# p-mc-grath/DMMFODS

Measured on AMD Instinct MI355X. Metric: training images/sec at 1280x1920 RGB+LiDAR, higher is better.
Workload: dtype f16; 1 GPU; C2 d121 early-fusion 6ch b4 1280x1920; key=c2, per_gpu_batch=4, global_batch=4, height=1280, width=1920, storage_dtype=fp16, accumulate=fp32, parallelism=dp1, weights=random-init (reference init, seed 123)

## Files before the change

dmmfods_amd/_lib.py:

```python
import ctypes as C
import os

_HERE = os.path.dirname(os.path.abspath(__file__))
LIB_PATH = os.environ.get("DMM_LIB_PATH") or os.path.join(_HERE, "libdmmfods_hip.so")

DMM_F32, DMM_F16, DMM_BF16 = 0, 1, 2
LOSS_BCE, LOSS_FOCAL = 0, 1
T_CONV, T_CONVT, T_BN_WEIGHT, T_BN_BIAS, T_BN_MEAN, T_BN_VAR, T_BN_TRACKED = range(7)
ERR_INVALID, ERR_SHAPE, ERR_HIP, ERR_STATE, ERR_NO_DEVICE = -1, -2, -3, -4, -5


class ModelDesc(C.Structure):
    _fields_ = [
        ("growth_rate", C.c_int32), ("num_blocks", C.c_int32), ("block_config", C.c_int32 * 8),
        ("num_init_features", C.c_int32), ("bn_size", C.c_int32), ("num_classes", C.c_int32),
        ("concat_before_block_num", C.c_int32), ("stream_1_in_channels", C.c_int32),
        ("stream_2_in_channels", C.c_int32), ("batch", C.c_int32), ("height", C.c_int32), ("width", C.c_int32),
        ("dtype", C.c_int32), ("loss_scale", C.c_float), ("bn_momentum", C.c_float), ("bn_eps", C.c_float),
        ("iou_threshold", C.c_float), ("use_mfma", C.c_int32),
    ]


class ConvDesc(C.Structure):
    _fields_ = [(n, C.c_int32) for n in (
# ... 24 lines not shown
    if not os.path.exists(LIB_PATH):
        raise ImportError(
            f"{LIB_PATH} is missing: build it with `python -c 'import __graft_entry__ as g; g.build()'` "
            "(or `make -C dmmfods_amd/csrc`).  dmmfods_amd has no CPU fallback.")
    import torch
    tl = os.path.join(os.path.dirname(torch.__file__), "lib", "libamdhip64.so")
    if os.path.exists(tl):
        C.CDLL(tl, mode=C.RTLD_GLOBAL)
    L = C.CDLL(LIB_PATH)
    vp, i32, i64, f32, sz = C.c_void_p, C.c_int32, C.c_int64, C.c_float, C.c_size_t
    L.dmm_last_error.restype = C.c_char_p
    L.dmm_version.restype = C.c_int
    L.dmm_last_impl.restype = C.c_int
    L.dmm_impl_name.restype = C.c_char_p
    L.dmm_impl_name.argtypes = [C.c_int]
    L.dmm_impl_mask.restype = C.c_uint
    L.dmm_impl_mask.argtypes = [C.c_int]
    L.dmm_set_option.restype = C.c_int
    L.dmm_set_option.argtypes = [C.c_char_p, C.c_int]
    L.dmm_plan_create.argtypes = [C.POINTER(ModelDesc), C.POINTER(vp)]
    L.dmm_plan_destroy.argtypes = [vp]
    L.dmm_plan_destroy.restype = C.c_int
    L.dmm_plan_num_tensors.argtypes = [vp]
    L.dmm_plan_tensor_info.argtypes = [vp, C.c_int, C.POINTER(C.c_char_p), C.POINTER(i32), C.POINTER(i32),
                                       C.POINTER(i64 * 4), C.POINTER(i64)]
    L.dmm_plan_num_params.argtypes = [vp]
    L.dmm_plan_num_params.restype = i64
    L.dmm_plan_num_buffer_elems.argtypes = [vp]
    L.dmm_plan_num_buffer_elems.restype = i64
    L.dmm_plan_workspace_bytes.argtypes = [vp]
# ... 33 lines not shown
    L.dmm_conv_wgrad_ex.argtypes = [C.POINTER(ConvDesc), vp, vp, vp, vp, vp, vp, vp, C.c_int, vp, vp, vp]
    L.dmm_conv_dgrad_ex.argtypes = [C.POINTER(ConvDesc), vp, vp, vp, vp, vp, vp, vp, vp, vp, C.c_int, vp, vp, vp]
    L.dmm_conv1x1_backward_fused.argtypes = [C.POINTER(ConvDesc), vp, vp, vp, vp, vp, vp, vp, vp, vp, C.c_int, vp, vp, vp, vp]
    L.dmm_conv5_wgrad_stats.argtypes = [C.POINTER(ConvDesc), vp, vp, vp, vp, vp, vp, vp, vp, vp]
    _lib = L
    return L


EXPORTS = [
    "dmm_last_error", "dmm_version", "dmm_set_option", "dmm_plan_create", "dmm_plan_destroy", "dmm_plan_num_tensors",
    "dmm_plan_tensor_info", "dmm_plan_num_params", "dmm_plan_num_buffer_elems", "dmm_plan_workspace_bytes",
    "dmm_plan_forward_flops", "dmm_plan_bind", "dmm_plan_forward", "dmm_plan_loss_backward", "dmm_plan_backward",
    "dmm_plan_loss_metrics", "dmm_plan_num_graph_replays", "dmm_plan_set_loss", "dmm_loss_forward", "dmm_plan_num_grad_buckets", "dmm_plan_grad_bucket",
    "dmm_plan_grad_bucket_wait", "dmm_plan_profile_begin", "dmm_plan_profile_filter", "dmm_plan_profile_num_ops", "dmm_plan_profile_op",
    "dmm_plan_profile_collect", "dmm_adam_step", "dmm_conv_scratch_bytes", "dmm_conv_forward", "dmm_conv_wgrad",
    "dmm_conv_dgrad", "dmm_conv_wgrad_ex", "dmm_conv_dgrad_ex", "dmm_conv1x1_backward_fused", "dmm_conv5_wgrad_stats", "dmm_last_impl", "dmm_impl_name", "dmm_impl_mask",
    "dmm_grad_guard_scratch_bytes", "dmm_guard_state_init", "dmm_adam_step_guarded", "dmm_grad_sumsq", "dmm_plan_set_dynamic_loss_scale",
]


def check(rc):
    if rc == 0:
        return
    msg = lib().dmm_last_error().decode(errors="replace")
    if rc == ERR_SHAPE:
        raise ValueError(msg)
    if rc == ERR_INVALID and "fusion" in msg:
        raise AttributeError(msg)
    if rc == ERR_INVALID:
        raise ValueError(msg)
    raise DmmError(f"dmm status {rc}: {msg}")
# ... 17 lines not shown
```

dmmfods_amd/csrc/capi.cpp:

```cpp
#include <algorithm>
#include <atomic>
#include <cmath>
#include <cstdio>
#include <cstdlib>
#include <cstring>
#include <stdexcept>
#include <chrono>
#include <mutex>
#include <string>
#include <unistd.h>

#include "dispatch.h"
#include "plan.h"

using namespace dmm;

void plan_build_tables(dmm_plan* p);
void plan_bind(dmm_plan* p, void* ws);

static thread_local std::string g_err;
static int fail(int code, const std::string& msg) {
  g_err = msg;
  return code;
}
#define HIPCHK(expr)                                                                                   \
  do {                                                                                                 \
    hipError_t e__ = (expr);                                                                           \
    if (e__ != hipSuccess) return fail(DMM_ERR_HIP, std::string(#expr) + ": " + hipGetErrorString(e__)); \
  } while (0)

static bool g_overlap_wgrad = getenv("DMM_NO_OVERLAP") == nullptr;
static int g_graph = getenv("DMM_GRAPH") ? std::max(1, atoi(getenv("DMM_GRAPH"))) : 0;
static unsigned long long g_option_epoch = 1;
static int g_bucket_mb = getenv("DMM_GRAD_BUCKET_MB") ? atoi(getenv("DMM_GRAD_BUCKET_MB")) : 25;
static std::atomic<unsigned> g_family_off{lab_family_off()};
static unsigned plan_deny(const dmm_plan* p) { return (p->sw.no_hf ? 1u << IMPL_HF : 0u) | g_family_off; }

namespace {
struct DevicePool {
  std::mutex mu;
  hipStream_t side = nullptr, pack = nullptr, capture = nullptr;
  std::vector<hipEvent_t> free_plain, free_timing;
  long events_made = 0;
};
constexpr int MAX_DEVICES = 64;
DevicePool* g_pools[MAX_DEVICES] = {};
std::mutex g_pools_mu;

DevicePool* pool_of(int device) {
  if (device < 0 || device >= MAX_DEVICES) return nullptr;
// ... 49 lines not shown

const char* dmm_last_error(void) { return g_err.c_str(); }
int dmm_version(void) { return 101; }

static const char* const kImplNames[IMPL_COUNT] = {"auto", "generic", "thin", "conv3", "cvp", "halo", "wg3", "wg5", "wgp", "pig", "bw1", "hf", "cf", "wgpw", "cvw"};
static const struct { const char* option; int family; } kFamilyOptions[] = {
    {"thin_logits", IMPL_THIN}, {"conv3", IMPL_CONV3}, {"wg3", IMPL_WG3}, {"wgp", IMPL_WGP},
    {"wg5", IMPL_WG5},          {"cvp", IMPL_CVP},     {"bw1", IMPL_BW1}, {"pig", IMPL_PIG},
};

int dmm_set_option(const char* name, int value) {
  if (!name) return fail(DMM_ERR_INVALID, "null argument");
  ++g_option_epoch;
  if (std::string(name) == "overlap_wgrad") { g_overlap_wgrad = value != 0; return DMM_OK; }
  if (std::string(name) == "graph") { g_graph = value; return DMM_OK; }
  for (const auto& o : kFamilyOptions)
    if (std::string(name) == o.option) {
      if (value != 0) g_family_off &= ~(1u << o.family);
      else g_family_off |= 1u << o.family;
      return DMM_OK;
    }
  if (std::string(name) == "grad_bucket_mb") {
    if (value < 0) return fail(DMM_ERR_INVALID, "grad_bucket_mb must be >= 0");
    g_bucket_mb = value;
    return DMM_OK;
  }
  return fail(DMM_ERR_INVALID, std::string("unknown option ") + name);
}

int dmm_plan_create(const dmm_model_desc* desc, dmm_plan** out) {
// ... 655 lines not shown
  const size_t dg = (size_t)((d->R * d->S * rup(d->Cout, 8) + g.BK - 1) / g.BK + 16) * rup(d->Cin, 128) * g.BK * g.esz;
  return fwd + dg + 2 * dg + (size_t)rup(d->Cout, 8) * 8 + 8192 + (size_t)W5_SBUF64_FLOATS * sizeof(float);
}

static void fill_one_seg(Seg& s, const dmm_conv_desc* d, const OneConv& g, const void* x, const float* scale, const float* shift,
                         const std::vector<Tap>& taps) {
  memset(&s, 0, sizeof(s));
  s.src = x; s.ld = g.Cst; s.Hs = d->H; s.Ws = d->W; s.C = g.Cst; s.Cpad = g.Cst;
  s.mode = d->transposed ? 0 : d->mode;
  s.istride = g.istride;
  if (d->bn_relu) { s.scale = scale; s.shift = shift; }
  fill_seg_taps(s, taps, g.BK);
}

int dmm_last_impl(void) { return g_last_impl; }
unsigned dmm_impl_mask(int reset) { const unsigned m = g_impl_mask; if (reset) g_impl_mask = 0; return m; }
const char* dmm_impl_name(int impl) { return impl >= 0 && impl < IMPL_COUNT ? kImplNames[impl] : "?"; }

int dmm_conv_forward(const dmm_conv_desc* d, const void* x, const float* w, const float* scale, const float* shift, void* y,
                     double* stats, void* scratch, void* stream) {
  OneConv g;
  if (!d || !geometry(d, g)) return fail(DMM_ERR_INVALID, "unsupported conv descriptor");
  hipStream_t st = (hipStream_t)stream;
  std::vector<PackDesc> packs;
  std::vector<int> prefix;
  PackDesc* dd; int* dp; int total_rows;
  layout_fwd(d, g, (uint8_t*)scratch, w, nullptr, packs, &dd, &dp, prefix, total_rows);
  HIPCHK(upload(dd, packs.data(), packs.size() * sizeof(PackDesc), st));
  HIPCHK(upload(dp, prefix.data(), prefix.size() * sizeof(int), st));
  HIPCHK(hipStreamSynchronize(st));
// ... 84 lines not shown
    HIPCHK(hipMemsetAsync(dw, 0, wn * sizeof(float), st));
    HIPCHK(launch_unpack(dd, dp, 1, pd.seg[0].nchunks * pd.Npad, d->dtype, 1.0f, st));
    return DMM_OK;
  }
  std::vector<PackDesc> packs;
  std::vector<int> prefix;
  PackDesc* dd; int* dp; int total_rows;
  const size_t used = layout_fwd(d, g, (uint8_t*)scratch, dw , dw, packs, &dd, &dp, prefix, total_rows);
  Scratch S{(uint8_t*)scratch, used};
  float* zeros = (float*)S.take((size_t)rup(d->Cout, 8) * sizeof(float) + 64);
  if (S.off > dmm_conv_scratch_bytes(d)) return fail(DMM_ERR_INVALID, "scratch too small");
  HIPCHK(hipMemsetAsync(scratch, 0, S.off, st));
  HIPCHK(upload(dd, packs.data(), packs.size() * sizeof(PackDesc), st));
  HIPCHK(upload(dp, prefix.data(), prefix.size() * sizeof(int), st));
  HIPCHK(hipStreamSynchronize(st));
  for (size_t ph = 0; ph < packs.size(); ++ph) {
    WgradArgs a;
    memset(&a, 0, sizeof(a));
    a.nseg = 1;
    fill_one_seg(a.seg[0], d, g, x, scale, shift, g.phase_taps[ph]);
    a.B = d->B; a.Ho = g.Ho; a.Wo = g.Wo; a.M = d->B * g.Ho * g.Wo;
    a.dy.src = dy; a.dy.ld = d->Cout; a.dy.Hs = g.Hout; a.dy.Ws = g.Wout; a.dy.C = rup(d->Cout, 8); a.dy.Cpad = a.dy.C;
    a.dy.mode = G_PLAIN; a.dy.istride = g.ostride; a.dy.ntaps = 1; a.dy.nchunks = 1;
    a.dy.taps[0] = (short)((g.phase_xy[ph].first & 0xff) | ((g.phase_xy[ph].second & 0xff) << 8));
    set_eff_grad(a.dy, yfwd, d->Cout, q, r, zeros);
    a.N = d->Cout; a.Npad = packs[ph].Npad;
    a.dpack = (float*)packs[ph].dpack;
    HIPCHK(launch_wgrad(a, d->dtype, d->use_mfma != 0, st, IMPL_AUTO, g_family_off));
  }
  HIPCHK(hipMemsetAsync(dw, 0, wn * sizeof(float), st));
  HIPCHK(launch_unpack(dd, dp, (int)packs.size(), total_rows, d->dtype, 1.0f, st));
  return DMM_OK;
}

int dmm_conv5_wgrad_stats(const dmm_conv_desc* d, const void* x, const void* dy, const float* w, const float* scale, const float* shift,
                          float* dw, double* red, void* scratch, void* stream) {
  OneConv g;
  if (!d || !geometry(d, g)) return fail(DMM_ERR_INVALID, "unsupported conv descriptor");
  if (d->transposed || d->mode != 0 || d->stride != 1 || d->R != 5 || d->S != 5 || d->pad != 2 || !d->bn_relu || d->Cin != 64 || d->Cout > 4 ||
      d->dtype == DMM_F32 || !d->use_mfma)
    return fail(DMM_ERR_INVALID, "serves the 5x5 convolution of 64 channels onto <= 4 behind BN+ReLU in 16-bit storage");
  hipStream_t st = (hipStream_t)stream;
  const size_t wn = (size_t)d->Cin * d->Cout * 25;
  const std::vector<Tap> taps = taps_conv_dgrad(5, 5, 2);
// ... 161 lines not shown
```

dmmfods_amd/csrc/common.h:

```cpp
#pragma once
#include <hip/hip_runtime.h>
#include <stddef.h>
#include <stdint.h>
#include <stdlib.h>

namespace dmm {

typedef _Float16 f16;
typedef f16 f16x8 __attribute__((ext_vector_type(8)));
typedef f16 f16x4 __attribute__((ext_vector_type(4)));
typedef __bf16 bf16;
typedef bf16 bf16x8 __attribute__((ext_vector_type(8)));
typedef bf16 bf16x4 __attribute__((ext_vector_type(4)));
typedef bf16 bf16x2 __attribute__((ext_vector_type(2)));
typedef float f32x4 __attribute__((ext_vector_type(4)));
typedef float f32x16 __attribute__((ext_vector_type(16)));

enum DType { DT_F32 = 0, DT_F16 = 1, DT_BF16 = 2 };
static inline size_t dtype_size(int dt) { return dt == DT_F32 ? 4 : 2; }

template <typename T> struct TT;
template <> struct TT<float> {
  static constexpr int SLOT = 4;
  typedef f32x4 vec;
// ... 80 lines not shown
  Seg dy;
  int N, Npad;
  float* dpack;
  int rows_per_split;
  int kgroups;
  float* part;
  int part_slots;
  int nphase;
  short ph_xtaps[4][4];
  short ph_ytap[4];
  float* ph_dpack[4];
  const float* t_mean;
  const float* t_invstd;
  float* sbuf;
  signed char ph_ntaps[4];
};
struct RawFinArgs {
  const float* sbuf;
  float* dpack;
  int Npad;
  const float* w;
  int Kin, koff, nreal;
  int tapw[9];
  const float* gamma;
  const float* beta;
  double* red1;
  double* red2;
};
constexpr int W5_SBUF_FLOATS = 5 * 64 * 32;
struct Fin64Args {
  const float* sbuf;
// ... 63 lines not shown
```

dmmfods_amd/csrc/plan.cpp:

```cpp
#include "plan.h"

#include <algorithm>
#include <cmath>
#include <cstdio>
#include <cstdlib>
#include <cstring>
#include <map>
#include <stdexcept>

namespace dmm {

static unsigned tw1(int mt) { return 0xffffff00u | (unsigned)mt; }

std::vector<Tap> taps_conv(int R, int S, int pad) {
  std::vector<Tap> t;
  for (int ky = 0; ky < R; ++ky)
    for (int kx = 0; kx < S; ++kx) t.push_back({ky - pad, kx - pad, tw1(ky * S + kx)});
  return t;
}
std::vector<Tap> taps_conv_dgrad(int R, int S, int pad) {
  std::vector<Tap> t;
  for (int ky = 0; ky < R; ++ky)
    for (int kx = 0; kx < S; ++kx) t.push_back({pad - ky, pad - kx, tw1(ky * S + kx)});
  return t;
// ... 741 lines not shown
      const PackDesc& pd = P.packs[ph.pack];
      a.N = c.N; a.Npad = pd.Npad;
      a.dpack = (float*)pd.dpack;
      const double np = (double)c.phases.size();
      o.impl = wgrad_pick(a, dtype, d.use_mfma != 0, deny);
      tag(o, ncls(o.impl, ROLE_WGRAD, pd.Npad), short_name(c.wname), conv_flops(c, c.phases.size()) * (wseg < c.nseg ? (double)c.seg[0].Cw / c.Kin : 1.0),
          (src_bytes(c) + grad_reads(c) * out_bytes(c)) / np + w_bytes(c) * 4.0 / esz / np);
    }
    if (c.phases.size() == 4 && wseg == 1 && !P.sw.no_wgp_merge)
      merge_last_four_phases(
          [](const Op& po, const Op& f) {
            const int nt = po.w.seg[0].ntaps;
            return po.kind == OP_WGRAD && po.impl == IMPL_WGP && po.w.nseg == 1 && (nt == 1 || nt == 2 || nt == 4) && po.w.seg[0].src == f.w.seg[0].src &&
                   po.w.dy.src == f.w.dy.src;
          },
          [](Op& m, const Op& po, int ph) {
            m.w.nphase = 4;
            for (int t = 0; t < 4; ++t) m.w.ph_xtaps[ph][t] = po.w.seg[0].taps[t < po.w.seg[0].ntaps ? t : 0];
            m.w.ph_ntaps[ph] = (signed char)po.w.seg[0].ntaps;
            m.w.ph_ytap[ph] = po.w.dy.taps[0];
            m.w.ph_dpack[ph] = po.w.dpack;
          },
          [&](Op& m) {
            bool all4 = true;
            for (int ph = 0; ph < 4; ++ph) all4 = all4 && m.w.ph_ntaps[ph] == 4;
            if (all4) m.w.ph_ntaps[0] = m.w.ph_ntaps[1] = m.w.ph_ntaps[2] = m.w.ph_ntaps[3] = 0;
            return wgrad_pick(m.w, dtype, d.use_mfma != 0, deny) == IMPL_WGP;
          });
  }

  bool raw_segment_once(const ConvRec& c) const {
    return c.nseg == 2 && c.phases.size() == 4 && c.shared_master && c.seg[1].C == 8 && c.seg[1].istride == 2 && c.ostride == 2 &&
           !lab_flag("DMM_NO_RAW_ONCE");
  }
  void emit_wgrad_raw(ConvRec& c, ConvBwd& st) {
    const Buf& ob = bufs[c.obuf];
    const SegRec& sr = c.seg[1];
    float* raw_sbuf = nullptr;
    if (dtype != DT_F32 && c.N == 64 && !P.sw.no_raw_stats) raw_sbuf = zbptr<float>(W5_SBUF_FLOATS);
    Op& o = push(OP_WGRAD);
    WgradArgs& a = o.w;
// ... 711 lines not shown
};

}
}

using namespace dmm;

PlanSwitches PlanSwitches::from_environment() {
  PlanSwitches s;
  auto on = [](const char* n) { const char* v = getenv(n); return v != nullptr && !(v[0] == '0' && v[1] == 0); };
  s.no_pack_tiles = on("DMM_NO_PACK_TILES");
  s.no_hf = on("DMM_NO_HF");
  s.no_c3_merge = on("DMM_NO_C3_MERGE");
  s.no_cvp_merge = on("DMM_NO_CVP_MERGE");
  s.no_wgp_merge = on("DMM_NO_WGP_MERGE");
  s.no_two_pass = on("DMM_NO_TWO_PASS");
  s.no_eff_compact = on("DMM_NO_EFF_COMPACT");
  s.no_s2_interleave = on("DMM_NO_S2_INTERLEAVE");
  s.no_raw_stats = on("DMM_NO_RAW_STATS");
  s.no_r1_stats = on("DMM_NO_R1_STATS");
  const char* pc = getenv("DMM_PACK_CUT");
  s.pack_cut = pc ? std::max(1, atoi(pc)) : 0;
  return s;
}

void plan_build_tables(dmm_plan* p) {
  build_tensor_table(p->desc, p->tensors, p->nparams, p->nbuf);
  Builder b(*p, true, nullptr);
  b.build();
  b.emit_all();
// ... 39 lines not shown
```

dmmfods_amd/csrc/plan.h:

```cpp
#pragma once
#include <cstring>
#include <stdexcept>
#include <string>
#include <vector>

#include "../../include/dmmfods_hip.h"
#include "common.h"
#include "pointwise.h"

namespace dmm {

struct plan_sizing_error : std::runtime_error { using std::runtime_error::runtime_error; };

struct TensorInfo {
  std::string name;
  int kind, ndim;
  int64_t shape[4];
  int64_t off;
};

struct Tap {
  int dy, dx;
  unsigned tapw;
};
// ... 45 lines not shown
    RawFinArgs rf;
    Fin64Args f64;
  };
  Op() { memset(static_cast<void*>(this), 0, sizeof(*this)); signal = -1; impl = IMPL_AUTO; }
};

}

struct GradBucket {
  int64_t off = 0, n = 0;
  int ev_main = -1, ev_side = -1;
  int ready = -1;
};

struct PlanSwitches {
  bool no_pack_tiles = false, no_hf = false, no_c3_merge = false, no_cvp_merge = false, no_wgp_merge = false, no_two_pass = false,
       no_eff_compact = false, no_s2_interleave = false, no_raw_stats = false, no_r1_stats = false;
  int pack_cut = 0;
  static PlanSwitches from_environment();
};

struct dmm_plan {
  dmm_model_desc desc;
  PlanSwitches sw;
  unsigned deny = 0;
  std::vector<dmm::TensorInfo> tensors;
  int64_t nparams = 0, nbuf = 0;
  size_t zero_bytes = 0, zero_bwd_bytes = 0, main_bytes = 0;
  double fwd_flops = 0;
  bool bound = false;
  void* ws = nullptr;
// ... 42 lines not shown
```

dmmfods_amd/csrc/wgp.hip:

```cpp
#include <algorithm>
#include <cstdio>
#include <cstdlib>

#include "common.h"
#include "dispatch.h"
#include "gather.h"
#include "isa.h"

namespace dmm {

constexpr int WP_TH = 8, WP_TW = 16;
constexpr int WP_HH = 9, WP_HWR = 17;
constexpr int WP_HW = 20;
constexpr int WP_CA = 128;
constexpr int WP_X_BYTES = WP_HH * WP_HW * 256;
constexpr int WP_Y_BYTES = BM * 256;
constexpr int WP_LDS = WP_X_BYTES + WP_Y_BYTES;

struct WgpArgs {
  WgradArgs w;
  int tiles_y, tiles_x, ntiles, tiles_per_wg, nsplit;
  int nct, ncot;
  int dymin, dxmin;
  int ph_dymin[4], ph_dxmin[4];
// ... 175 lines not shown
  const int r = lane & 31, h = lane >> 5;
  const int cpt = sx.Cpad / 32;
#pragma unroll
  for (int t = 0; t < NTAP; ++t) {
    const size_t chunk = (size_t)t * cpt + ct * 4 + wave;
#pragma unroll
    for (int j = 0; j < NJ; ++j)
#pragma unroll
      for (int i = 0; i < 16; ++i) {
        const int n = cot * NCO + 32 * j + (i & 3) + 8 * (i >> 2) + 4 * h;
        atomic_add_f32(dpack_ + (chunk * a.Npad + n) * 32 + r, acc[t][j][i]);
      }
  }
}

bool wgpw_resolve(const WgradArgs& a, int dtype, int ntap, int nj, const WgpGeom& q, Resolved& r);
hipError_t wgpw_launch(const Resolved& r, hipStream_t st);

template <typename T>
static LdsLauncher<WgpArgs> wgp_instance(int ntap, int nj, int pq) {
  if (ntap == 4 && nj == 2) return pq ? launch_lds<wgp_kernel<T, 4, 2, 2>, WgpArgs> : launch_lds<wgp_kernel<T, 4, 2, 0>, WgpArgs>;
  if (ntap == 2 && nj == 4) return pq ? launch_lds<wgp_kernel<T, 2, 4, 2>, WgpArgs> : launch_lds<wgp_kernel<T, 2, 4, 0>, WgpArgs>;
  if (ntap == 2 && nj == 2) return pq ? launch_lds<wgp_kernel<T, 2, 2, 2>, WgpArgs> : launch_lds<wgp_kernel<T, 2, 2, 0>, WgpArgs>;
  return nullptr;
}

struct WgpLaunch {
  WgpArgs g;
  LdsLauncher<WgpArgs> run;
};
// ... 76 lines not shown
hipError_t wgp_launch(const Resolved& r, hipStream_t st) {
  static const bool trace = lab_flag("DMM_WGP_TRACE");
  if (trace) {
    const WgradArgs& a = r.get<WgradArgs>();
    const Seg &x = a.seg[0], &y = a.dy;
    fprintf(stderr, "wgp? nseg %d x: mode %d istride %d Hs %d Ws %d (Ho %d Wo %d) scale %d C %d Cpad %d ntaps %d | y: mode %d ntaps %d istride %d Hs %d Ws %d C %d | N %d Npad %d\n",
            a.nseg, x.mode, x.istride, x.Hs, x.Ws, a.Ho, a.Wo, x.scale != nullptr, x.C, x.Cpad, x.ntaps, y.mode, y.ntaps, y.istride, y.Hs, y.Ws, y.C, a.N, a.Npad);
  }
  if (r.form == IMPL_WGPW) {
    note_impl(IMPL_WGPW);
    return wgpw_launch(r, st);
  }
  const WgpLaunch& l = r.get<WgpLaunch>();
  WgpArgs g = l.g;
  const int nwg = wgp_split(g.ntiles, g.nct, g.ncot, g.w.nphase, g.tiles_per_wg, g.nsplit);
  if (trace) fprintf(stderr, "wgp: ntap %d nj %d pq %d pairs %d nsplit %d tiles/wg %d\n", g.w.seg[0].ntaps, g.w.N / (32 * g.ncot), g.w.dy.q ? 2 : 0, g.nct * g.ncot, g.nsplit, g.tiles_per_wg);
  return l.run(WP_LDS, nwg, NTHREADS, WP_LDS, st, g);
}

}
```

dmmfods_amd/csrc/wgpw.hip:

```cpp
#include <algorithm>
#include <cstdio>
#include <cstdlib>

#include "common.h"
#include "dispatch.h"
#include "gather.h"
#include "isa.h"

namespace dmm {

constexpr int WW_TH = 8, WW_TW = 16;
constexpr int WW_HH = 9, WW_HWR = 17, WW_HW = 20;
constexpr int WW_CA = 128;
constexpr int WW_X_BYTES = WW_HH * WW_HW * 256;
constexpr int WW_Y_BYTES = BM * 256;
constexpr int WW_LDS = 2 * (WW_X_BYTES + WW_Y_BYTES);
constexpr int WW_Y0 = 2 * WW_X_BYTES;
static_assert(WW_X_BYTES < 65536 && WW_Y_BYTES < 65536, "set offsets fit the instruction's immediate");
constexpr int WW_NT = 512;
static_assert(WW_LDS <= 160 * 1024, "two image sets fit the LDS of a compute unit");

struct WgpwArgs {
  WgradArgs w;
  int tiles_y, tiles_x, ntiles, tiles_per_wg, nsplit;
  int nct, ncot;
  int dymin, dxmin;
  int ph_dymin[4], ph_dxmin[4];
};

constexpr int WW_NX = 10;
template <typename V, int NY, int MODE>
__device__ __forceinline__ void ww_sync(V (&rx)[WW_NX], V (&ry)[NY]) {
  static_assert(WW_NX == 10 && (NY == 4 || NY == 8), "DMM_V10 and DMM_V4 / DMM_V8 below");
  if constexpr (NY == 4) {
    if constexpr (MODE == 2) DMM_VM_HOLD(DMM_V10(rx), DMM_V4(ry));
    else DMM_VM_WAIT(MODE == 0 ? WW_NX + NY : 0, DMM_V10(rx), DMM_V4(ry));
  } else {
    if constexpr (MODE == 2) DMM_VM_HOLD(DMM_V10(rx), DMM_V8(ry));
    else DMM_VM_WAIT(MODE == 0 ? WW_NX + NY : 0, DMM_V10(rx), DMM_V8(ry));
  }
}

struct WgpwPhase { int dymin, dxmin, ytap; float* dpack; short xt0, xt1, xt2, xt3; };

template <typename T, int NTAP, int NJ>
__device__ __forceinline__ void wgpw_body(const WgpwArgs& g, const int unit, const WgpwPhase P) {
  static_assert(sizeof(T) == 2, "16-bit storage");
  typedef typename TT<T>::vec V;
  constexpr int SLOT = 8;
  constexpr int NL = 256;
  constexpr int NCO = 32 * NJ;
  constexpr int NX = WW_NX;
  constexpr int YS = NCO / SLOT;
  constexpr int NY = BM * YS / NL;
  constexpr int YRS = NL / YS;
  static_assert(WW_HH * WW_HWR * (WW_CA / SLOT) <= NX * NL, "halo slots covered");
  const WgradArgs& a = g.w;
  const Seg& sx = a.seg[0];
  const Seg& sy = a.dy;

  extern __shared__ __attribute__((aligned(16))) unsigned char smem[];
  const int tid = threadIdx.x, lane = tid & 63, wave = tid >> 6;
  if (unit >= g.nsplit * g.nct * g.ncot) return;
  const int pair = unit % (g.nct * g.ncot), split = unit / (g.nct * g.ncot);
  const int ct = pair % g.nct, cot = pair / g.nct;
  const int dymin_ = P.dymin, dxmin_ = P.dxmin, ytap_ = P.ytap;
  float* const dpack_ = P.dpack;
  const short xt0 = P.xt0, xt1 = P.xt1, xt2 = P.xt2, xt3 = P.xt3;
  const int t_beg = split * g.tiles_per_wg, t_end = min(g.ntiles, t_beg + g.tiles_per_wg);
  if (t_beg >= t_end) return;
  const int nt = t_end - t_beg;
  const int tiles_img = g.tiles_y * g.tiles_x;

  if (wave >= 4) {
    const int lt = tid - NL;
    const int cx = lt & 15, px0 = lt >> 4;
    const int cy = lt % YS, py0 = lt / YS;
    SlotK<SLOT> kx;
    kx.k0 = load_fv<SLOT>(sx.scale + ct * WW_CA + cx * SLOT); kx.k1 = load_fv<SLOT>(sx.shift + ct * WW_CA + cx * SLOT); kx.k2 = 0.f; kx.k3 = 0.f;
    const unsigned xcol = (unsigned)(ct * WW_CA + cx * SLOT) * 2u, ycol = (unsigned)(cot * NCO + cy * SLOT) * 2u;
    const unsigned xpitch = (unsigned)sx.ld * 2u, ypitch = (unsigned)sy.ld * 2u;
    const int ypy = (int)(signed char)(ytap_ & 0xff), ypx = (int)(signed char)((ytap_ >> 8) & 0xff);
    int xlds[NX];
    unsigned xrel[NX];
    unsigned xin = 0;
#pragma unroll
    for (int i = 0; i < NX; ++i) {
      const int hp = px0 + 16 * i;
      const int hpc = min(hp, WW_HH * WW_HWR - 1);
      const int hy = hpc / WW_HWR, hx = hpc - hy * WW_HWR;
      if (hp < WW_HH * WW_HWR) xin |= 1u << i;
      const int idx = hy * WW_HW + hx;
      xlds[i] = idx * 256 + ((cx * 16) ^ ((idx & 3) << 6));
      xrel[i] = (unsigned)(hy * sx.Ws + hx) * xpitch + xcol;
    }
    static_assert(YRS % 4 == 0, "the swizzle key (pixel & 3) of a thread's dY slots is that of its first");
// ... 82 lines not shown
      store(R1, 1);
      lds_barrier();
      __builtin_amdgcn_sched_barrier(0);
      issue(R1);
      __builtin_amdgcn_sched_barrier(0);
    }
    ww_sync<V, NY, 1>(R0.rx, R0.ry);
    ww_sync<V, NY, 2>(R1.rx, R1.ry);
    if (nt & 1) {
      store(R0, 0, false);
      lds_barrier();
    }
    return;
  }

  f32x16 acc[NTAP][NJ];
#pragma unroll
  for (int t = 0; t < NTAP; ++t)
#pragma unroll
    for (int j = 0; j < NJ; ++j)
#pragma unroll
      for (int i = 0; i < 16; ++i) acc[t][j][i] = 0.f;

  const int tg = lane >> 4, ti = lane & 15, tq = ti >> 2, tp = ti & 3;
  const int arow = 8 * (tg >> 1) + tq;
  const int xcolb = (32 * wave + 16 * (tg & 1) + 4 * tp) * 2;
  int xoff[NTAP];
#pragma unroll
  for (int t = 0; t < NTAP; ++t) {
    const int tw = t == 0 ? xt0 : (t == 1 ? xt1 : (t == 2 ? xt2 : xt3));
// ... 54 lines not shown
  const int unit = (slot8 >> 2) * 8 + (blockIdx.x & 7);
  WgpwPhase P = {g.ph_dymin[0], g.ph_dxmin[0], g.w.ph_ytap[0], g.w.ph_dpack[0], g.w.ph_xtaps[0][0], g.w.ph_xtaps[0][1], g.w.ph_xtaps[0][2], g.w.ph_xtaps[0][3]};
  int nt = g.w.ph_ntaps[0];
#pragma unroll
  for (int q = 1; q < 4; ++q)
    if (q == ph) {
      P.dymin = g.ph_dymin[q]; P.dxmin = g.ph_dxmin[q]; P.ytap = g.w.ph_ytap[q]; P.dpack = g.w.ph_dpack[q];
      P.xt0 = g.w.ph_xtaps[q][0]; P.xt1 = g.w.ph_xtaps[q][1]; P.xt2 = g.w.ph_xtaps[q][2]; P.xt3 = g.w.ph_xtaps[q][3];
      nt = g.w.ph_ntaps[q];
    }
  if (nt == 0 || nt == 4) wgpw_body<T, 4, 2>(g, unit, P);
  else if (nt == 2) wgpw_body<T, 2, 2>(g, unit, P);
  else wgpw_body<T, 1, 2>(g, unit, P);
}

struct WgpwLaunch {
  WgpwArgs g;
  LdsLauncher<WgpwArgs> run;
};
int wgp_split(int ntiles, int nct, int ncot, int nphase, int& tiles_per_wg, int& nsplit);

bool wgpw_resolve(const WgradArgs& a, int dtype, int ntap, int nj, const WgpGeom& q, Resolved& r) {
  if ((double)a.B * a.seg[0].Hs * a.seg[0].Ws * a.seg[0].ld * 2.0 >= 4294967296.0 || (double)a.B * a.dy.Hs * a.dy.Ws * a.dy.ld * 2.0 >= 4294967296.0)
    return false;
  WgpwLaunch& l = r.put<WgpwLaunch>();
  WgpwArgs& g = l.g;
  g.w = a;
  g.tiles_y = q.tiles_y; g.tiles_x = q.tiles_x; g.ntiles = q.ntiles; g.nct = q.nct; g.ncot = q.ncot; g.dymin = q.dymin; g.dxmin = q.dxmin;
  for (int ph = 0; ph < 4; ++ph) { g.ph_dymin[ph] = q.ph_dymin[ph]; g.ph_dxmin[ph] = q.ph_dxmin[ph]; }
  const bool f = dtype == DT_F16;
  l.run = nullptr;
  if (a.nphase == 4 && nj == 2) l.run = f ? launch_lds<wgpw_multi_kernel<f16>, WgpwArgs> : launch_lds<wgpw_multi_kernel<bf16>, WgpwArgs>;
  else if (a.nphase != 0) return false;
  else if (ntap == 4 && nj == 2) l.run = f ? launch_lds<wgpw_kernel<f16, 4, 2>, WgpwArgs> : launch_lds<wgpw_kernel<bf16, 4, 2>, WgpwArgs>;
  else if (ntap == 2 && nj == 4) l.run = f ? launch_lds<wgpw_kernel<f16, 2, 4>, WgpwArgs> : launch_lds<wgpw_kernel<bf16, 2, 4>, WgpwArgs>;
  else if (ntap == 2 && nj == 2) l.run = f ? launch_lds<wgpw_kernel<f16, 2, 2>, WgpwArgs> : launch_lds<wgpw_kernel<bf16, 2, 2>, WgpwArgs>;
  else if (ntap == 1 && nj == 4) l.run = f ? launch_lds<wgpw_kernel<f16, 1, 4>, WgpwArgs> : launch_lds<wgpw_kernel<bf16, 1, 4>, WgpwArgs>;
  else if (ntap == 1 && nj == 2) l.run = f ? launch_lds<wgpw_kernel<f16, 1, 2>, WgpwArgs> : launch_lds<wgpw_kernel<bf16, 1, 2>, WgpwArgs>;
  return l.run != nullptr;
}

hipError_t wgpw_launch(const Resolved& r, hipStream_t st) {
  WgpwArgs g = r.get<WgpwLaunch>().g;
  const int nwg = wgp_split(g.ntiles, g.nct, g.ncot, g.w.nphase, g.tiles_per_wg, g.nsplit);
  return r.get<WgpwLaunch>().run(WW_LDS, nwg, WW_NT, WW_LDS, st, g);
}

}
```

include/dmmfods_hip.h:

```cpp
#ifndef DMMFODS_HIP_H
#define DMMFODS_HIP_H
#include <stddef.h>
#include <stdint.h>

#ifdef __cplusplus
extern "C" {
#endif

typedef enum {
  DMM_OK = 0,
  DMM_ERR_INVALID = -1,
  DMM_ERR_SHAPE = -2,
  DMM_ERR_HIP = -3,
  DMM_ERR_STATE = -4,
  DMM_ERR_NO_DEVICE = -5
} dmm_status;

enum { DMM_F32 = 0, DMM_F16 = 1, DMM_BF16 = 2 };

enum { DMM_T_CONV = 0, DMM_T_CONVT = 1, DMM_T_BN_WEIGHT = 2, DMM_T_BN_BIAS = 3, DMM_T_BN_MEAN = 4, DMM_T_BN_VAR = 5,
       DMM_T_BN_TRACKED = 6 };

typedef struct {
  int32_t growth_rate;
// ... 106 lines not shown

int dmm_conv_wgrad_ex(const dmm_conv_desc* d, const void* x, const void* dy, const float* scale, const float* shift, const void* yfwd,
                      const float* q, const float* r, int transposed_form, float* dw, void* scratch, void* stream);
int dmm_conv_dgrad_ex(const dmm_conv_desc* d, const void* x, const void* dy, const float* w, const float* scale, const float* shift,
                      const void* yfwd, const float* q, const float* r, void* gx, int accumulate, double* red, void* scratch,
                      void* stream);
int dmm_conv5_wgrad_stats(const dmm_conv_desc* d, const void* x, const void* dy, const float* w, const float* scale, const float* shift,
                          float* dw, double* red, void* scratch, void* stream);
int dmm_conv1x1_backward_fused(const dmm_conv_desc* d, const void* x, const void* dy, const float* w, const float* scale,
                               const float* shift, const void* yfwd, const float* q, const float* r, void* gx, int accumulate,
                               float* dw, double* red, void* scratch, void* stream);

int dmm_last_impl(void);
const char* dmm_impl_name(int impl);
unsigned dmm_impl_mask(int reset);

#ifdef __cplusplus
}
#endif
#endif
```

Before: 159.3 img/s.

## Add quad-phase wgrad kernel sharing Y/X fragments across four transposed-conv phases

Adds a QUAD variant of the wgpw weight-gradient kernel. When the four phase-decomposed wgrad passes of a stride-2 transposed conv form a 1/2/2/4 tap pattern inside one 2x2 box, a single workgroup loads all four phases' dy columns and the four X box fragments once, then computes the 9 distinct (phase, tap) products. This replaces the old multi-phase path, which split the phases across workgroups and reloaded X. The quad path is on by default in the plan merge (disable with DMM_NO_WGP_QUAD); a standalone API option to merge phases is also added, off by default. The cost is 9 accumulator tiles per wave, which raises register pressure, and a different work split.

```diff
diff --git a/dmmfods_amd/_lib.py b/dmmfods_amd/_lib.py
--- a/dmmfods_amd/_lib.py
+++ b/dmmfods_amd/_lib.py
@@ -62,6 +62,7 @@
     L.dmm_last_impl.restype = C.c_int
     L.dmm_impl_name.restype = C.c_char_p
     L.dmm_impl_name.argtypes = [C.c_int]
+    L.dmm_last_wgp_kernel.restype = C.c_char_p
     L.dmm_impl_mask.restype = C.c_uint
     L.dmm_impl_mask.argtypes = [C.c_int]
     L.dmm_set_option.restype = C.c_int
@@ -125,7 +126,7 @@
     "dmm_plan_loss_metrics", "dmm_plan_num_graph_replays", "dmm_plan_set_loss", "dmm_loss_forward", "dmm_plan_num_grad_buckets", "dmm_plan_grad_bucket",
     "dmm_plan_grad_bucket_wait", "dmm_plan_profile_begin", "dmm_plan_profile_filter", "dmm_plan_profile_num_ops", "dmm_plan_profile_op",
     "dmm_plan_profile_collect", "dmm_adam_step", "dmm_conv_scratch_bytes", "dmm_conv_forward", "dmm_conv_wgrad",
-    "dmm_conv_dgrad", "dmm_conv_wgrad_ex", "dmm_conv_dgrad_ex", "dmm_conv1x1_backward_fused", "dmm_conv5_wgrad_stats", "dmm_last_impl", "dmm_impl_name", "dmm_impl_mask",
+    "dmm_conv_dgrad", "dmm_conv_wgrad_ex", "dmm_conv_dgrad_ex", "dmm_conv1x1_backward_fused", "dmm_conv5_wgrad_stats", "dmm_last_impl", "dmm_impl_name", "dmm_impl_mask", "dmm_last_wgp_kernel",
     "dmm_grad_guard_scratch_bytes", "dmm_guard_state_init", "dmm_adam_step_guarded", "dmm_grad_sumsq", "dmm_plan_set_dynamic_loss_scale",
 ]
 
diff --git a/dmmfods_amd/csrc/capi.cpp b/dmmfods_amd/csrc/capi.cpp
--- a/dmmfods_amd/csrc/capi.cpp
+++ b/dmmfods_amd/csrc/capi.cpp
@@ -34,6 +34,8 @@
 static unsigned long long g_option_epoch = 1;
 static int g_bucket_mb = getenv("DMM_GRAD_BUCKET_MB") ? atoi(getenv("DMM_GRAD_BUCKET_MB")) : 25;
 static std::atomic<unsigned> g_family_off{lab_family_off()};
+namespace dmm { extern thread_local const char* g_last_wgp_kernel; }
+static bool g_wgrad_merge_phases = false;
 static unsigned plan_deny(const dmm_plan* p) { return (p->sw.no_hf ? 1u << IMPL_HF : 0u) | g_family_off; }
 
 namespace {
@@ -113,6 +115,7 @@
   ++g_option_epoch;
   if (std::string(name) == "overlap_wgrad") { g_overlap_wgrad = value != 0; return DMM_OK; }
   if (std::string(name) == "graph") { g_graph = value; return DMM_OK; }
+  if (std::string(name) == "wgrad_merge_phases") { g_wgrad_merge_phases = value != 0; return DMM_OK; }
   for (const auto& o : kFamilyOptions)
     if (std::string(name) == o.option) {
       if (value != 0) g_family_off &= ~(1u << o.family);
@@ -798,6 +801,7 @@
 }
 
 int dmm_last_impl(void) { return g_last_impl; }
+const char* dmm_last_wgp_kernel(void) { return g_last_wgp_kernel; }
 unsigned dmm_impl_mask(int reset) { const unsigned m = g_impl_mask; if (reset) g_impl_mask = 0; return m; }
 const char* dmm_impl_name(int impl) { return impl >= 0 && impl < IMPL_COUNT ? kImplNames[impl] : "?"; }
 
@@ -912,8 +916,9 @@
   HIPCHK(upload(dd, packs.data(), packs.size() * sizeof(PackDesc), st));
   HIPCHK(upload(dp, prefix.data(), prefix.size() * sizeof(int), st));
   HIPCHK(hipStreamSynchronize(st));
+  std::vector<WgradArgs> phases(packs.size());
   for (size_t ph = 0; ph < packs.size(); ++ph) {
-    WgradArgs a;
+    WgradArgs& a = phases[ph];
     memset(&a, 0, sizeof(a));
     a.nseg = 1;
     fill_one_seg(a.seg[0], d, g, x, scale, shift, g.phase_taps[ph]);
@@ -924,8 +929,24 @@
     set_eff_grad(a.dy, yfwd, d->Cout, q, r, zeros);
     a.N = d->Cout; a.Npad = packs[ph].Npad;
     a.dpack = (float*)packs[ph].dpack;
-    HIPCHK(launch_wgrad(a, d->dtype, d->use_mfma != 0, st, IMPL_AUTO, g_family_off));
-  }
+  }
+  bool merged = false;
+  const unsigned deny = g_family_off;
+  if (g_wgrad_merge_phases && phases.size() == 4) {
+    bool each = true;
+    for (const WgradArgs& a : phases) each = each && wgrad_pick(a, d->dtype, d->use_mfma != 0, deny) == IMPL_WGP;
+    if (each) {
+      WgradArgs m = phases[0];
+      for (int ph = 0; ph < 4; ++ph) wgrad_merge_phase(m, phases[ph], ph);
+      wgrad_merge_done(m);
+      if (wgrad_pick(m, d->dtype, d->use_mfma != 0, deny) == IMPL_WGP) {
+        HIPCHK(launch_wgrad(m, d->dtype, d->use_mfma != 0, st, IMPL_WGP, deny));
+        merged = true;
+      }
+    }
+  }
+  if (!merged)
+    for (const WgradArgs& a : phases) HIPCHK(launch_wgrad(a, d->dtype, d->use_mfma != 0, st, IMPL_AUTO, deny));
   HIPCHK(hipMemsetAsync(dw, 0, wn * sizeof(float), st));
   HIPCHK(launch_unpack(dd, dp, (int)packs.size(), total_rows, d->dtype, 1.0f, st));
   return DMM_OK;
diff --git a/dmmfods_amd/csrc/common.h b/dmmfods_amd/csrc/common.h
--- a/dmmfods_amd/csrc/common.h
+++ b/dmmfods_amd/csrc/common.h
@@ -118,7 +118,20 @@
   const float* t_invstd;
   float* sbuf;
   signed char ph_ntaps[4];
-};
+  signed char ph_split_wgs;
+};
+inline void wgrad_merge_phase(WgradArgs& m, const WgradArgs& po, int ph) {
+  m.nphase = 4;
+  for (int t = 0; t < 4; ++t) m.ph_xtaps[ph][t] = po.seg[0].taps[t < po.seg[0].ntaps ? t : 0];
+  m.ph_ntaps[ph] = (signed char)po.seg[0].ntaps;
+  m.ph_ytap[ph] = po.dy.taps[0];
+  m.ph_dpack[ph] = po.dpack;
+}
+inline void wgrad_merge_done(WgradArgs& m) {
+  bool all4 = true;
+  for (int ph = 0; ph < 4; ++ph) all4 = all4 && m.ph_ntaps[ph] == 4;
+  if (all4) m.ph_ntaps[0] = m.ph_ntaps[1] = m.ph_ntaps[2] = m.ph_ntaps[3] = 0;
+}
 struct RawFinArgs {
   const float* sbuf;
   float* dpack;
diff --git a/dmmfods_amd/csrc/plan.cpp b/dmmfods_amd/csrc/plan.cpp
--- a/dmmfods_amd/csrc/plan.cpp
+++ b/dmmfods_amd/csrc/plan.cpp
@@ -779,17 +779,12 @@
             return po.kind == OP_WGRAD && po.impl == IMPL_WGP && po.w.nseg == 1 && (nt == 1 || nt == 2 || nt == 4) && po.w.seg[0].src == f.w.seg[0].src &&
                    po.w.dy.src == f.w.dy.src;
           },
-          [](Op& m, const Op& po, int ph) {
-            m.w.nphase = 4;
-            for (int t = 0; t < 4; ++t) m.w.ph_xtaps[ph][t] = po.w.seg[0].taps[t < po.w.seg[0].ntaps ? t : 0];
-            m.w.ph_ntaps[ph] = (signed char)po.w.seg[0].ntaps;
-            m.w.ph_ytap[ph] = po.w.dy.taps[0];
-            m.w.ph_dpack[ph] = po.w.dpack;
+          [&](Op& m, const Op& po, int ph) {
+            wgrad_merge_phase(m.w, po.w, ph);
+            m.w.ph_split_wgs = P.sw.no_wgp_quad;
           },
           [&](Op& m) {
-            bool all4 = true;
-            for (int ph = 0; ph < 4; ++ph) all4 = all4 && m.w.ph_ntaps[ph] == 4;
-            if (all4) m.w.ph_ntaps[0] = m.w.ph_ntaps[1] = m.w.ph_ntaps[2] = m.w.ph_ntaps[3] = 0;
+            wgrad_merge_done(m.w);
             return wgrad_pick(m.w, dtype, d.use_mfma != 0, deny) == IMPL_WGP;
           });
   }
@@ -1531,6 +1526,7 @@
   s.no_c3_merge = on("DMM_NO_C3_MERGE");
   s.no_cvp_merge = on("DMM_NO_CVP_MERGE");
   s.no_wgp_merge = on("DMM_NO_WGP_MERGE");
+  s.no_wgp_quad = on("DMM_NO_WGP_QUAD");
   s.no_two_pass = on("DMM_NO_TWO_PASS");
   s.no_eff_compact = on("DMM_NO_EFF_COMPACT");
   s.no_s2_interleave = on("DMM_NO_S2_INTERLEAVE");
diff --git a/dmmfods_amd/csrc/plan.h b/dmmfods_amd/csrc/plan.h
--- a/dmmfods_amd/csrc/plan.h
+++ b/dmmfods_amd/csrc/plan.h
@@ -83,7 +83,7 @@
 };
 
 struct PlanSwitches {
-  bool no_pack_tiles = false, no_hf = false, no_c3_merge = false, no_cvp_merge = false, no_wgp_merge = false, no_two_pass = false,
+  bool no_pack_tiles = false, no_hf = false, no_c3_merge = false, no_cvp_merge = false, no_wgp_merge = false, no_wgp_quad = false, no_two_pass = false,
        no_eff_compact = false, no_s2_interleave = false, no_raw_stats = false, no_r1_stats = false;
   int pack_cut = 0;
   static PlanSwitches from_environment();
diff --git a/dmmfods_amd/csrc/wgp.hip b/dmmfods_amd/csrc/wgp.hip
--- a/dmmfods_amd/csrc/wgp.hip
+++ b/dmmfods_amd/csrc/wgp.hip
@@ -213,6 +213,7 @@
   }
 }
 
+thread_local const char* g_last_wgp_kernel = "";
 bool wgpw_resolve(const WgradArgs& a, int dtype, int ntap, int nj, const WgpGeom& q, Resolved& r);
 hipError_t wgpw_launch(const Resolved& r, hipStream_t st);
 
@@ -319,6 +320,7 @@
   const WgpLaunch& l = r.get<WgpLaunch>();
   WgpArgs g = l.g;
   const int nwg = wgp_split(g.ntiles, g.nct, g.ncot, g.w.nphase, g.tiles_per_wg, g.nsplit);
+  g_last_wgp_kernel = "wgp";
   if (trace) fprintf(stderr, "wgp: ntap %d nj %d pq %d pairs %d nsplit %d tiles/wg %d\n", g.w.seg[0].ntaps, g.w.N / (32 * g.ncot), g.w.dy.q ? 2 : 0, g.nct * g.ncot, g.nsplit, g.tiles_per_wg);
   return l.run(WP_LDS, nwg, NTHREADS, WP_LDS, st, g);
 }
diff --git a/dmmfods_amd/csrc/wgpw.hip b/dmmfods_amd/csrc/wgpw.hip
--- a/dmmfods_amd/csrc/wgpw.hip
+++ b/dmmfods_amd/csrc/wgpw.hip
@@ -26,7 +26,12 @@
   int nct, ncot;
   int dymin, dxmin;
   int ph_dymin[4], ph_dxmin[4];
+  short q_box[4];
+  signed char q_tap[12];
 };
+constexpr int WQ_ACC = 9;
+__device__ __host__ constexpr int wq_slot(int a) { return a < 1 ? 0 : (a < 3 ? 1 : (a < 5 ? 2 : 3)); }
+__device__ __host__ constexpr int wq_box(int a) { return a < 1 ? 0 : (a < 3 ? a - 1 : (a < 5 ? 2 * (a - 3) : a - 5)); }
 
 constexpr int WW_NX = 10;
 template <typename V, int NY, int MODE>
@@ -43,15 +48,16 @@
 
 struct WgpwPhase { int dymin, dxmin, ytap; float* dpack; short xt0, xt1, xt2, xt3; };
 
-template <typename T, int NTAP, int NJ>
+template <typename T, int NTAP, int NJ, bool QUAD = false>
 __device__ __forceinline__ void wgpw_body(const WgpwArgs& g, const int unit, const WgpwPhase P) {
   static_assert(sizeof(T) == 2, "16-bit storage");
   typedef typename TT<T>::vec V;
   constexpr int SLOT = 8;
   constexpr int NL = 256;
-  constexpr int NCO = 32 * NJ;
+  constexpr int NCO = QUAD ? 32 : 32 * NJ;
+  static_assert(!QUAD || NJ == 4, "four phase slots");
   constexpr int NX = WW_NX;
-  constexpr int YS = NCO / SLOT;
+  constexpr int YS = 32 * NJ / SLOT;
   constexpr int NY = BM * YS / NL;
   constexpr int YRS = NL / YS;
   static_assert(WW_HH * WW_HWR * (WW_CA / SLOT) <= NX * NL, "halo slots covered");
@@ -64,7 +70,7 @@
   if (unit >= g.nsplit * g.nct * g.ncot) return;
   const int pair = unit % (g.nct * g.ncot), split = unit / (g.nct * g.ncot);
   const int ct = pair % g.nct, cot = pair / g.nct;
-  const int dymin_ = P.dymin, dxmin_ = P.dxmin, ytap_ = P.ytap;
+  const int dymin_ = P.dymin, dxmin_ = P.dxmin;
   float* const dpack_ = P.dpack;
   const short xt0 = P.xt0, xt1 = P.xt1, xt2 = P.xt2, xt3 = P.xt3;
   const int t_beg = split * g.tiles_per_wg, t_end = min(g.ntiles, t_beg + g.tiles_per_wg);
@@ -78,8 +84,13 @@
     const int cy = lt % YS, py0 = lt / YS;
     SlotK<SLOT> kx;
     kx.k0 = load_fv<SLOT>(sx.scale + ct * WW_CA + cx * SLOT); kx.k1 = load_fv<SLOT>(sx.shift + ct * WW_CA + cx * SLOT); kx.k2 = 0.f; kx.k3 = 0.f;
-    const unsigned xcol = (unsigned)(ct * WW_CA + cx * SLOT) * 2u, ycol = (unsigned)(cot * NCO + cy * SLOT) * 2u;
+    const unsigned xcol = (unsigned)(ct * WW_CA + cx * SLOT) * 2u, ycol = (unsigned)(cot * NCO + (QUAD ? cy & 3 : cy) * SLOT) * 2u;
     const unsigned xpitch = (unsigned)sx.ld * 2u, ypitch = (unsigned)sy.ld * 2u;
+    int ytap_ = P.ytap;
+    if constexpr (QUAD) {
+#pragma unroll
+      for (int q = 1; q < 4; ++q) if ((cy >> 2) == q) ytap_ = g.w.ph_ytap[q];
+    }
     const int ypy = (int)(signed char)(ytap_ & 0xff), ypx = (int)(signed char)((ytap_ >> 8) & 0xff);
     int xlds[NX];
     unsigned xrel[NX];
@@ -192,6 +203,55 @@
     return;
   }
 
+  if constexpr (QUAD) {
+    f32x16 acc[WQ_ACC];
+#pragma unroll
+    for (int a = 0; a < WQ_ACC; ++a)
+#pragma unroll
+      for (int i = 0; i < 16; ++i) acc[a][i] = 0.f;
+    const int tg = lane >> 4, ti = lane & 15, tq = ti >> 2, tp = ti & 3;
+    const int arow = 8 * (tg >> 1) + tq;
+    const int xcolb = (32 * wave + 16 * (tg & 1) + 4 * tp) * 2;
+    int xoff[4], yoff[4];
+#pragma unroll
+    for (int b = 0; b < 4; ++b) {
+      const int tw = g.q_box[b];
+      const int idx = (tw & 0xff) * WW_HW + arow + ((tw >> 8) & 0xff);
+      xoff[b] = idx * 256 + (xcolb ^ ((idx & 3) << 6));
+      yoff[b] = arow * 256 + (((32 * b + 16 * (tg & 1) + 4 * tp) * 2) ^ (tq << 6));
+    }
+    for (int k = 0; k < nt; ++k) {
+      lds_barrier();
+      const unsigned char* Xs = smem + (k & 1) * WW_X_BYTES;
+      const unsigned char* Ys = smem + WW_Y0 + (k & 1) * WW_Y_BYTES;
+#pragma unroll 2
+      for (int ms = 0; ms < WW_TH; ++ms) {
+        const unsigned char* yp = Ys + ms * (16 * 256);
+        const unsigned char* xp = Xs + ms * (WW_HW * 256);
+        V yf[4], xf[4];
+#pragma unroll
+        for (int b = 0; b < 4; ++b) {
+          yf[b] = frag16<T>(lds_tr16(yp + yoff[b]), lds_tr16(yp + yoff[b] + 4 * 256));
+          xf[b] = frag16<T>(lds_tr16(xp + xoff[b]), lds_tr16(xp + xoff[b] + 4 * 256));
+        }
+#pragma unroll
+        for (int a = 0; a < WQ_ACC; ++a) acc[a] = mma16(yf[wq_slot(a)], xf[wq_box(a)], acc[a]);
+      }
+    }
+    const int r = lane & 31, h = lane >> 5;
+    const int cpt = sx.Cpad / 32;
+#pragma unroll
+    for (int a = 0; a < WQ_ACC; ++a) {
+      float* const dp = g.w.ph_dpack[wq_slot(a)];
+      const size_t chunk = (size_t)g.q_tap[a] * cpt + ct * 4 + wave;
+#pragma unroll
+      for (int i = 0; i < 16; ++i) {
+        const int n = cot * NCO + (i & 3) + 8 * (i >> 2) + 4 * h;
+        atomic_add_f32(dp + (chunk * g.w.Npad + n) * 32 + r, acc[a][i]);
+      }
+    }
+    return;
+  }
   f32x16 acc[NTAP][NJ];
 #pragma unroll
   for (int t = 0; t < NTAP; ++t)
@@ -276,10 +336,68 @@
   else wgpw_body<T, 1, 2>(g, unit, P);
 }
 
+template <typename T>
+__global__ __launch_bounds__(WW_NT, 1) void wgpw_quad_kernel(const WgpwArgs g) {
+  const WgpwPhase P = {g.dymin, g.dxmin, g.w.ph_ytap[0], nullptr, 0, 0, 0, 0};
+  wgpw_body<T, 4, 4, true>(g, blockIdx.x, P);
+}
+
 struct WgpwLaunch {
   WgpwArgs g;
   LdsLauncher<WgpwArgs> run;
+  bool quad;
 };
+
+bool wgpw_quad_order(const WgradArgs& a, WgpwArgs& g) {
+  if (a.nphase != 4) return false;
+  int slot[4], n1 = 0, n2 = 0, n4 = 0;
+  for (int ph = 0; ph < 4; ++ph) {
+    const int nt = a.ph_ntaps[ph];
+    if (nt == 1 && n1 == 0) { slot[0] = ph; ++n1; }
+    else if (nt == 2 && n2 < 2) { slot[1 + n2] = ph; ++n2; }
+    else if (nt == 4 && n4 == 0) { slot[3] = ph; ++n4; }
+    else return false;
+  }
+  int ymin = 127, xmin = 127;
+  for (int ph = 0; ph < 4; ++ph)
+    for (int t = 0; t < a.ph_ntaps[ph]; ++t) {
+      ymin = std::min(ymin, (int)(signed char)(a.ph_xtaps[ph][t] & 0xff));
+      xmin = std::min(xmin, (int)(signed char)((a.ph_xtaps[ph][t] >> 8) & 0xff));
+    }
+  int box[4][4];
+  unsigned set[4] = {0, 0, 0, 0};
+  for (int s = 0; s < 4; ++s)
+    for (int t = 0; t < a.ph_ntaps[slot[s]]; ++t) {
+      const short tw = a.ph_xtaps[slot[s]][t];
+      const int dy = (int)(signed char)(tw & 0xff) - ymin, dx = (int)(signed char)((tw >> 8) & 0xff) - xmin;
+      if (dy > 1 || dx > 1) return false;
+      box[s][t] = dy * 2 + dx;
+      if (set[s] & (1u << box[s][t])) return false;
+      set[s] |= 1u << box[s][t];
+    }
+  const unsigned b0 = set[0];
+  if (!(set[1] & b0) || !(set[2] & b0) || set[1] == set[2] || set[3] != 15u) return false;
+  const unsigned order[4] = {b0, set[1] & ~b0, set[2] & ~b0, 15u & ~(set[1] | set[2])};
+  for (int k = 0; k < 4; ++k) {
+    int bi = 0;
+    while (!((order[k] >> bi) & 1u)) ++bi;
+    g.q_box[k] = (short)((bi >> 1) | ((bi & 1) << 8));
+  }
+  for (int i = 0; i < 12; ++i) g.q_tap[i] = 0;
+  for (int i = 0; i < WQ_ACC; ++i) {
+    const int s = wq_slot(i);
+    int t = 0;
+    while (!((order[wq_box(i)] >> box[s][t]) & 1u)) ++t;
+    g.q_tap[i] = (signed char)t;
+  }
+  for (int s = 0; s < 4; ++s) {
+    const int ph = slot[s];
+    for (int t = 0; t < 4; ++t) g.w.ph_xtaps[s][t] = a.ph_xtaps[ph][t];
+    g.w.ph_ytap[s] = a.ph_ytap[ph]; g.w.ph_dpack[s] = a.ph_dpack[ph]; g.w.ph_ntaps[s] = a.ph_ntaps[ph];
+  }
+  g.dymin = ymin; g.dxmin = xmin;
+  return true;
+}
 int wgp_split(int ntiles, int nct, int ncot, int nphase, int& tiles_per_wg, int& nsplit);
 
 bool wgpw_resolve(const WgradArgs& a, int dtype, int ntap, int nj, const WgpGeom& q, Resolved& r) {
@@ -292,7 +410,11 @@
   for (int ph = 0; ph < 4; ++ph) { g.ph_dymin[ph] = q.ph_dymin[ph]; g.ph_dxmin[ph] = q.ph_dxmin[ph]; }
   const bool f = dtype == DT_F16;
   l.run = nullptr;
-  if (a.nphase == 4 && nj == 2) l.run = f ? launch_lds<wgpw_multi_kernel<f16>, WgpwArgs> : launch_lds<wgpw_multi_kernel<bf16>, WgpwArgs>;
+  l.quad = a.nphase == 4 && !a.ph_split_wgs && wgpw_quad_order(a, g);
+  if (l.quad) {
+    g.ncot = a.N / 32;
+    l.run = f ? launch_lds<wgpw_quad_kernel<f16>, WgpwArgs> : launch_lds<wgpw_quad_kernel<bf16>, WgpwArgs>;
+  } else if (a.nphase == 4 && nj == 2) l.run = f ? launch_lds<wgpw_multi_kernel<f16>, WgpwArgs> : launch_lds<wgpw_multi_kernel<bf16>, WgpwArgs>;
   else if (a.nphase != 0) return false;
   else if (ntap == 4 && nj == 2) l.run = f ? launch_lds<wgpw_kernel<f16, 4, 2>, WgpwArgs> : launch_lds<wgpw_kernel<bf16, 4, 2>, WgpwArgs>;
   else if (ntap == 2 && nj == 4) l.run = f ? launch_lds<wgpw_kernel<f16, 2, 4>, WgpwArgs> : launch_lds<wgpw_kernel<bf16, 2, 4>, WgpwArgs>;
@@ -302,9 +424,11 @@
   return l.run != nullptr;
 }
 
+extern thread_local const char* g_last_wgp_kernel;
 hipError_t wgpw_launch(const Resolved& r, hipStream_t st) {
   WgpwArgs g = r.get<WgpwLaunch>().g;
-  const int nwg = wgp_split(g.ntiles, g.nct, g.ncot, g.w.nphase, g.tiles_per_wg, g.nsplit);
+  g_last_wgp_kernel = r.get<WgpwLaunch>().quad ? "wgpw_quad" : (g.w.nphase == 4 ? "wgpw_multi" : "wgpw");
+  const int nwg = wgp_split(g.ntiles, g.nct, g.ncot, r.get<WgpwLaunch>().quad ? 0 : g.w.nphase, g.tiles_per_wg, g.nsplit);
   return r.get<WgpwLaunch>().run(WW_LDS, nwg, WW_NT, WW_LDS, st, g);
 }
 
diff --git a/include/dmmfods_hip.h b/include/dmmfods_hip.h
--- a/include/dmmfods_hip.h
+++ b/include/dmmfods_hip.h
@@ -144,6 +144,7 @@
 int dmm_last_impl(void);
 const char* dmm_impl_name(int impl);
 unsigned dmm_impl_mask(int reset);
+const char* dmm_last_wgp_kernel(void);
 
 #ifdef __cplusplus
 }
```

Result: no change. 160.6 img/s, median of 6 (+0.8%).
